# DavidPetrus/ood_object_detection

Measured on AMD Instinct MI355X. Metric: images/sec, tf_efficientdet_d0 640px bf16 inference + OOD score (DetBenchPredict end-to-end), higher is better.
Workload: dtype bf16; 1 GPU; tf_efficientdet_d0 640x640 batch=64/GPU C=90, DetBenchPredict: backbone+BiFPN+heads+OOD energy/max-logit+top-k(5000)+decode+hard NMS; global_batch=64, parallelism=image-sharded dp1, no collective, weights=seeded reference init, randomised BN stats, class bias 0, launch=hipgraph, images_in_flight=192

## Files before the change

ood_object_detection_amd/_lib.py:

```python
import ctypes
import os
import subprocess

_HERE = os.path.dirname(os.path.abspath(__file__))
LIB_PATH = os.path.join(_HERE, 'libeffdet_hip.so')
CSRC = os.path.join(_HERE, 'csrc')

_lib = None

LABEL_PAD = -2 ** 63

c_void_p, c_int, c_ll, c_float, c_double = ctypes.c_void_p, ctypes.c_int, ctypes.c_longlong, ctypes.c_float, ctypes.c_double
P = ctypes.POINTER

SIGNATURES = {
    'effdet_abi_version': (c_int, []),
    'effdet_last_error': (ctypes.c_char_p, []),
    'effdet_device_error': (c_int, [c_int]),
    'effdet_stem_conv': (c_int, [c_void_p, c_int, c_int, c_void_p, c_void_p, c_void_p, c_void_p, c_void_p,
                                 c_int, c_int, c_int, c_int]),
    'effdet_stem_dw_fused': (c_int, [c_void_p, c_int, c_int, c_void_p, c_void_p, c_void_p, c_void_p, c_void_p, c_void_p,
                                     c_void_p, c_void_p, c_void_p, c_int, c_int, c_int, c_int]),
    'effdet_resize_pad_u8': (c_int, [c_void_p, c_void_p, c_int, c_int, c_void_p, c_int, c_int, c_int, c_void_p, c_void_p, c_int,
                                     c_void_p, c_void_p, c_int, c_void_p, c_void_p]),
# ... 99 lines not shown
    'effdet_nms_soft_large': (c_int, [c_void_p, c_void_p, c_void_p, c_void_p, c_void_p, c_void_p, c_void_p, c_int, c_int,
                                      c_int, c_float, c_float, c_float, c_int, c_void_p, c_void_p, c_void_p, c_void_p, c_void_p]),
    'effdet_detection_loss_workspace_floats': (c_ll, [c_int, c_ll, c_int]),
    'effdet_detection_loss': (c_int, [c_void_p, c_int, c_void_p, c_void_p, c_void_p, c_void_p, c_void_p, c_int, c_ll, c_int,
                                      c_float, c_float, c_float, c_float, c_void_p, c_void_p, c_void_p, c_void_p, c_ll]),
    'effdet_label_anchors_workspace_bytes': (c_ll, [c_int, c_int, c_ll]),
    'effdet_label_anchors': (c_int, [c_void_p, c_void_p, c_void_p, c_void_p, c_int, c_int, c_ll, c_float, c_void_p, c_void_p,
                                     c_void_p, c_void_p, c_void_p, c_ll]),
    'effdet_label_anchors_rows': (c_int, [c_void_p, c_void_p, c_void_p, c_void_p, c_int, c_int, c_ll, c_float, c_void_p, c_void_p,
                                          c_void_p, c_void_p, c_void_p, c_ll]),
    'effdet_relabel_task_cls': (c_int, [c_void_p, c_void_p, c_void_p, c_int, c_int, c_ll, c_float]),
    'effdet_train_gemm_nt': (c_int, [c_void_p, c_void_p, c_ll, c_ll, c_ll, c_void_p, c_void_p, c_void_p, c_ll, c_ll, c_ll,
                                     c_ll, c_int, c_int, c_int, c_void_p]),
    'effdet_train_gemm_tn_workspace_floats': (c_ll, [c_ll, c_int, c_int]),
    'effdet_train_gemm_tn': (c_int, [c_void_p, c_void_p, c_ll, c_ll, c_ll, c_void_p, c_ll, c_ll, c_ll, c_ll, c_int, c_int,
                                     c_void_p, c_void_p, c_ll]),
    'effdet_train_reduce_mid': (c_int, [c_void_p, c_void_p, c_int, c_int, c_ll, c_void_p, c_int]),
    'effdet_train_dwconv_bwd_dx': (c_int, [c_void_p, c_void_p, c_void_p, c_void_p, c_int, c_int, c_int, c_int, c_int, c_int]),
    'effdet_train_dwconv_bwd_dw_workspace_floats': (c_ll, [c_int, c_int, c_int, c_int, c_int, c_int]),
    'effdet_train_dwconv_bwd_dw': (c_int, [c_void_p, c_void_p, c_void_p, c_void_p, c_int, c_int, c_int, c_int, c_int, c_int,
                                           c_void_p, c_ll, c_int]),
    'effdet_train_ew': (c_int, [c_void_p, c_int, c_void_p, c_void_p, c_void_p, c_void_p, c_void_p, c_void_p, c_void_p, c_void_p,
                                c_float, c_float, c_float, c_float, c_ll, c_int, c_ll, c_void_p, c_void_p]),
    'effdet_train_col_reduce_workspace_floats': (c_ll, [c_int, c_ll, c_int]),
    'effdet_train_col_reduce': (c_int, [c_void_p, c_int, c_void_p, c_void_p, c_void_p, c_int, c_ll, c_int, c_void_p, c_void_p, c_ll, c_float]),
    'effdet_train_spatial': (c_int, [c_void_p, c_int, c_void_p, c_void_p, c_void_p, c_int, c_int, c_int, c_int]),
    'effdet_train_im2col_stem': (c_int, [c_void_p, c_void_p, c_void_p, c_int, c_int, c_int]),
    'effdet_train_se_bwd': (c_int, [c_void_p, c_void_p, c_int, c_void_p, c_void_p, c_void_p, c_void_p, c_void_p, c_void_p, c_void_p,
                                    c_int, c_int, c_int]),
    'effdet_eval_match': (c_int, [c_void_p, c_void_p, c_void_p, c_void_p, c_void_p, c_int, c_int, c_int, c_int, c_float,
                                  c_void_p, c_void_p, c_void_p, c_void_p]),
    'effdet_eval_ap_workspace_bytes': (c_ll, [c_int]),
    'effdet_eval_ap': (c_int, [c_void_p, c_void_p, c_void_p, c_void_p, c_int, c_int, c_void_p, c_void_p, c_void_p, c_ll]),
    'effdet_eval_match_multi': (c_int, [c_void_p, c_void_p, c_void_p, c_void_p, c_void_p, c_void_p, c_int, c_int, c_int, c_int,
                                        c_void_p, c_int, c_void_p, c_void_p, c_void_p, c_void_p, c_void_p]),
    'effdet_eval_append': (c_int, [c_void_p, c_void_p, c_void_p, c_void_p, c_int, c_int, c_void_p, c_void_p, c_void_p, c_ll, c_void_p]),
    'effdet_eval_scale_sort_tile': (c_int, []),
    'effdet_eval_ap_sorted_workspace_bytes': (c_ll, [c_ll, c_int]),
    'effdet_eval_ap_sorted_offset': (c_ll, [c_ll, c_int, c_int]),
    'effdet_eval_ap_sorted_result_bytes': (c_ll, [c_int, c_int]),
    'effdet_eval_ap_sorted': (c_int, [c_void_p, c_void_p, c_void_p, c_void_p, c_ll, c_ll, c_void_p, c_int, c_int, c_void_p,
                                      c_void_p, c_void_p, c_void_p, c_ll, c_void_p]),
    'effdet_eval_open_words': (c_int, [c_void_p, c_void_p, c_void_p, c_void_p, c_void_p, c_int, c_int, c_int, c_int, c_void_p, c_int,
                                       c_void_p]),
    'effdet_eval_append_open': (c_int, [c_void_p, c_void_p, c_void_p, c_void_p, c_void_p, c_int, c_int, c_void_p, c_void_p, c_void_p,
                                        c_void_p, c_ll, c_void_p]),
    'effdet_eval_open_sorted_workspace_bytes': (c_ll, [c_ll, c_int]),
    'effdet_eval_open_sorted_offset': (c_ll, [c_ll, c_int, c_int]),
    'effdet_eval_open_sorted_result_bytes': (c_ll, [c_int, c_int]),
    'effdet_eval_open_sorted': (c_int, [c_void_p, c_void_p, c_void_p, c_void_p, c_void_p, c_ll, c_ll, c_void_p, c_int, c_int,
                                        c_void_p, c_void_p, c_void_p, c_double, c_void_p, c_ll, c_void_p]),
    'effdet_relabel_unknown': (c_int, [c_void_p, c_void_p, c_void_p, c_void_p, c_ll, c_ll, c_int, c_int, c_int, c_float, c_void_p,
                                       c_void_p]),
    'effdet_train_fold_bn': (c_int, [c_void_p, c_void_p, c_int, c_int, c_void_p, c_void_p, c_void_p, c_void_p, c_float,
                                     c_void_p, c_void_p, c_void_p, c_void_p, c_void_p, c_void_p]),
    'effdet_train_convbn_grads': (c_int, [c_void_p, c_void_p, c_int, c_int, c_int, c_void_p, c_void_p, c_void_p, c_void_p,
                                          c_void_p, c_void_p, c_void_p]),
    'effdet_train_bn_finalize': (c_int, [c_void_p, c_void_p, c_void_p, c_void_p, c_void_p, c_void_p, c_void_p, c_void_p, c_int, c_int,
                                         c_float, c_float, c_float, c_void_p, c_void_p, c_void_p]),
    'effdet_train_bn_bwd_prep': (c_int, [c_void_p, c_void_p, c_void_p, c_void_p, c_int, c_float, c_void_p, c_void_p, c_void_p, c_void_p]),
    'effdet_train_gemm_nt_levels': (c_int, [c_void_p, c_void_p, c_int, c_void_p, c_void_p, c_void_p, c_int, c_int, c_int, P(c_int), P(c_int),
                                            c_ll, c_ll, c_int, c_int, c_void_p]),
    'effdet_train_gemm_tn_levels': (c_int, [c_void_p, c_void_p, c_int, c_void_p, c_int, c_int, P(c_int), P(c_int), c_ll, c_ll, c_int, c_int,
                                            c_void_p, c_void_p, c_ll]),
    'effdet_train_levels_workspace_floats': (c_ll, [c_int, c_int, P(c_int), P(c_int), c_int]),
    'effdet_train_levels_dw': (c_int, [c_void_p, c_void_p, c_void_p, c_void_p, c_int, c_int, P(c_int), P(c_int), c_int, c_int]),
    'effdet_train_levels_dw_bwd_dw': (c_int, [c_void_p, c_void_p, c_void_p, c_void_p, c_int, c_int, P(c_int), P(c_int), c_int,
                                              c_void_p, c_ll, c_int]),
    'effdet_train_levels_col_reduce': (c_int, [c_void_p, c_int, c_void_p, c_void_p, c_void_p, c_void_p, P(c_float), c_int, c_int,
                                               P(c_int), P(c_int), c_int, c_void_p, c_void_p, c_ll]),
    'effdet_train_levels_bn_finalize': (c_int, [c_void_p, c_void_p, c_void_p, c_int, c_int, P(c_void_p), P(c_void_p), P(c_void_p),
                                                P(c_void_p), P(c_void_p), P(c_int), P(c_float), P(c_float), P(c_float), P(c_float),
                                                c_void_p, c_void_p, c_void_p, c_void_p]),
    'effdet_train_levels_bn_bwd_prep': (c_int, [c_void_p, c_void_p, c_void_p, P(c_float), c_int, c_int, c_void_p, c_void_p, c_void_p,
                                                c_void_p]),
    'effdet_train_levels_ew': (c_int, [c_void_p, c_int, c_void_p, c_void_p, c_void_p, c_void_p, c_void_p, c_void_p, c_void_p, c_void_p,
                                       c_void_p, P(c_int), c_int, c_int, P(c_int), P(c_int), c_int]),
    'effdet_train_fpn_weights': (c_int, [c_void_p, c_void_p, c_int, c_int, c_void_p]),
    'effdet_train_fpn_combine': (c_int, [c_void_p, c_int, P(c_void_p), P(c_int), P(c_int), c_int, c_void_p, c_void_p, c_void_p,
                                         c_int, c_int, c_int, c_int]),
    'effdet_train_fpn_dots_workspace_floats': (c_ll, [c_int, c_int, c_int, c_int]),
    'effdet_train_fpn_wgrad': (c_int, [c_void_p, c_int, P(c_void_p), P(c_int), P(c_int), c_int, c_void_p, c_void_p, c_void_p, c_void_p,
                                       c_void_p, c_void_p, c_int, c_int, c_int, c_int, c_void_p, c_ll]),
    'effdet_train_fpn_input_bwd': (c_int, [c_void_p, c_int, c_void_p, c_int, c_int, c_void_p, c_void_p, c_void_p, c_void_p, c_void_p,
                                           c_int, c_int, c_int, c_int]),
    'effdet_train_dwconv_fwd_parts': (c_int, [c_int, c_int, c_int, c_int, c_int]),
    'effdet_train_gemm_nt_plan_describe': (c_int, [c_ll, c_int, c_int, c_int, c_ll, c_ll, c_ll, c_int, c_ll, c_ll, c_ll, c_int, c_ll, c_int,
                                                   P(c_int), P(c_int), c_int]),
    'effdet_train_gemm_tn_plan_describe': (c_int, [c_ll, c_int, c_int, c_int, c_ll, c_ll, c_ll, c_int, c_ll, c_ll, c_ll, c_ll,
                                                   P(c_int), P(c_int), c_int]),
    'effdet_train_dwconv_plan_describe': (c_int, [c_int, c_int, c_int, c_int, c_int, c_int, c_int, P(c_int), c_int]),
    'effdet_train_dwconv_fwd': (c_int, [c_void_p, c_void_p, c_void_p, c_void_p, c_void_p, c_void_p, c_void_p, c_void_p,
                                        c_int, c_int, c_int, c_int, c_int, c_int]),
    'effdet_train_se_gate': (c_int, [c_void_p, c_void_p, c_int, c_int, c_void_p, c_void_p, c_void_p, c_void_p, c_void_p, c_void_p,
                                     c_int, c_int, c_int]),
    'effdet_train_gemm_nt_fused': (c_int, [c_void_p, c_void_p, c_void_p, c_ll, c_void_p, c_void_p, c_void_p, c_void_p, c_void_p,
                                           c_ll, c_int, c_int]),
    'effdet_train_gemm_tn_scaled': (c_int, [c_void_p, c_void_p, c_void_p, c_void_p, c_ll, c_ll, c_int, c_int, c_void_p, c_void_p, c_ll]),
    'effdet_train_dwconv_bwd_dx_silu': (c_int, [c_void_p, c_void_p, c_void_p, c_void_p, c_void_p, c_int, c_int, c_int, c_int, c_int, c_int]),
    'effdet_train_gemm_nt_relu': (c_int, [c_void_p, c_void_p, c_void_p, c_void_p, c_ll, c_int, c_int]),
    'effdet_train_gemm_nt_mask': (c_int, [c_void_p, c_void_p, c_void_p, c_void_p, c_void_p, c_ll, c_int, c_int]),
    'effdet_train_relu_mask': (c_int, [c_void_p, c_void_p, c_void_p, c_void_p, c_ll]),
    'effdet_train_prep_table': (c_int, [c_void_p, c_void_p, c_int, c_ll]),
    'effdet_train_grads_table': (c_int, [c_void_p, c_void_p, c_int, c_int]),
    'effdet_train_bn_var_finalize': (c_int, [c_void_p, c_void_p, c_void_p, c_ll, c_int, c_void_p, c_void_p, c_void_p, c_void_p, c_void_p,
                                             c_float, c_float, c_float, c_void_p, c_void_p, c_void_p, c_void_p, c_ll]),
    'effdet_train_bn_bwd_sums': (c_int, [c_void_p, c_void_p, c_void_p, c_void_p, c_void_p, c_ll, c_int, c_void_p, c_void_p, c_ll]),
    'effdet_gather_ood': (c_int, [c_void_p, c_void_p, c_void_p, c_void_p, c_void_p, c_ll, c_int, c_int, c_int,
                                  c_void_p, c_void_p, c_void_p]),
    'effdet_episode_select': (c_int, [c_void_p, c_int, c_int, P(c_void_p), P(c_ll), P(c_int), P(c_int), P(c_void_p)]),
    'effdet_episode_feed': (c_int, [c_void_p, c_int, c_int, P(c_void_p), P(c_ll), P(c_void_p), P(c_ll), P(c_void_p), P(c_int), P(c_int),
                                    c_void_p, c_void_p, c_int, c_void_p, c_int, c_int, c_int, c_int, c_int, c_void_p, c_void_p]),
    'effdet_episode_cluster_workspace_floats': (c_ll, [c_int, c_int, c_int]),
    'effdet_episode_cluster': (c_int, [c_void_p, c_void_p, c_void_p, c_int, c_int, c_int, c_float, c_float, c_void_p, c_int, c_float,
                                       c_int, c_void_p, c_ll, c_void_p, c_void_p, c_void_p, c_void_p, c_void_p, c_void_p, c_void_p,
                                       c_void_p, c_void_p, c_void_p, c_void_p]),
    'effdet_episode_proj_loss_workspace_floats': (c_ll, [c_int, c_int, c_int]),
    'effdet_episode_proj_loss': (c_int, [c_void_p, c_void_p, c_void_p, c_void_p, c_int, c_int, c_int, c_ll, c_void_p, c_float, c_float,
                                         c_void_p, c_void_p, c_void_p, c_void_p, c_void_p, c_int, c_int, c_float, c_void_p, c_ll,
                                         c_void_p, c_void_p, c_void_p, c_void_p]),
    'effdet_episode_proj_loss_backward': (c_int, [c_void_p, c_void_p, c_void_p, c_void_p, c_int, c_int, c_int, c_ll, c_void_p, c_float,
                                                  c_float, c_void_p, c_void_p, c_void_p, c_void_p, c_void_p, c_int, c_int, c_float,
                                                  c_void_p, c_void_p, c_ll, c_void_p, c_void_p, c_void_p]),
    'effdet_episode_supp_loss_workspace_floats': (c_ll, [c_int, c_int, c_int]),
    'effdet_episode_supp_loss': (c_int, [c_void_p, c_void_p, c_void_p, c_void_p, c_int, c_int, c_int, c_float, c_float, c_void_p,
                                         c_void_p, c_void_p, c_void_p, c_void_p, c_int, c_void_p, c_ll, c_void_p, c_void_p]),
    'effdet_episode_supp_loss_backward': (c_int, [c_void_p, c_void_p, c_void_p, c_void_p, c_int, c_int, c_int, c_float, c_float,
                                                  c_void_p, c_void_p, c_void_p, c_void_p, c_void_p, c_int, c_int, c_void_p, c_void_p,
                                                  c_ll, c_void_p, c_void_p, c_void_p, c_void_p]),
    'effdet_episode_supp_loss_backward2': (c_int, [c_void_p, c_void_p, c_void_p, c_void_p, c_int, c_int, c_int, c_float, c_float,
                                                   c_void_p, c_void_p, c_void_p, c_void_p, c_void_p, c_int, c_int, c_void_p, c_void_p,
                                                   c_void_p, c_void_p, c_void_p, c_void_p, c_void_p, c_ll, c_void_p, c_void_p,
                                                   c_void_p, c_void_p, c_void_p]),
    'effdet_inner_update_max_tensors': (c_int, []),
    'effdet_inner_update_max_step_sizes': (c_int, []),
    'effdet_inner_update_workspace_doubles': (c_ll, [c_int, P(c_ll)]),
    'effdet_inner_update': (c_int, [c_void_p, c_int, P(c_void_p), P(c_void_p), P(c_void_p), P(c_ll), P(c_int), c_int, P(c_void_p),
                                    P(c_float)]),
    'effdet_inner_update_backward': (c_int, [c_void_p, c_int, P(c_void_p), P(c_void_p), P(c_void_p), P(c_ll), P(c_int), c_int,
                                             P(c_void_p), P(c_float), c_void_p, c_ll, c_int, c_void_p]),
}


def build(verbose=False):
    jobs = str(min(8, os.cpu_count() or 1))
    r = subprocess.run(['make', '-C', CSRC, '-j', jobs], capture_output=not verbose, text=True)
    if r.returncode != 0:
        raise RuntimeError('building libeffdet_hip.so failed:\n%s\n%s' % (r.stdout, r.stderr))
    return LIB_PATH


TEST_VARIANTS = {
    'spin0': ('mbconv_wide', '-DWIDE_SPIN_LIMIT=0'),
}


def build_test_variants(verbose=False):
    paths = []
    for tag, (unit, defs) in TEST_VARIANTS.items():
        r = subprocess.run(['make', '-C', CSRC, 'variant', 'TAG=' + tag, 'UNIT=' + unit, 'VDEFS=' + defs], capture_output=not verbose, text=True)
        if r.returncode != 0:
            raise RuntimeError('building the %s variant failed:\n%s\n%s' % (tag, r.stdout, r.stderr))
        paths.append(os.path.join(_HERE, 'libeffdet_hip_%s.so' % tag))
    return paths


def load():
    global _lib
    if _lib is not None:
        return _lib
    import torch
    if not os.path.exists(LIB_PATH):
        raise RuntimeError('%s is missing - run `python -c "import __graft_entry__ as g; g.build()"` '
                           '(there is no CPU fallback for the HIP path)' % LIB_PATH)
    lib = ctypes.CDLL(LIB_PATH)
    for name, (res, args) in SIGNATURES.items():
        fn = getattr(lib, name)
        fn.restype = res
        fn.argtypes = args
    if lib.effdet_abi_version() != 1:
        raise RuntimeError('libeffdet_hip.so ABI version mismatch')
    _lib = lib
    return lib


def check(rc, what):
    if rc != 0:
        detail = ''
        if rc == -5 and _lib is not None:
            detail = ' (%s)' % (_lib.effdet_last_error() or b'').decode()
        raise RuntimeError('%s failed with code %d%s' % (what, rc, detail))
```

ood_object_detection_amd/csrc/sepconv.hip:

```cpp
#include "common.h"
#include <type_traits>

namespace {

struct SepInput {
    const void* ptr; long long image_stride;
    int H, W; int mode;
    int pad_t, pad_l;
};
struct SepLevel {
    int H, W, tiles_x, tiles_y, tile_begin, affine_row;
    SepInput in[3];
    void* out; long long out_image_stride;
    long long ood_off;
    int in_affine_row;
    void* dw_out; long long dw_out_image_stride;
};
struct SepArgs {
    int nlevels; SepLevel lv[5];
    int n_in, fuse_mode;
    float fw[3]; float fden;
    float fwn[3];
    int vec_ok;
    int out_f32;
    int pre_act, post_act;
    const float* dw_w;
    const void* pw_w;
    const float* scale; const float* shift;
    int F, N;
    int ood_classes, num_anchors;
    float* ood_energy; float* ood_maxlogit; long long ood_image_stride;
    const float* in_scale; const float* in_shift;
    float* stat_partial;
    int tiles_total;
};

constexpr int FC = 64;



template <typename T> struct Raw8 { u32x4 v[sizeof(T) == 2 ? 1 : 2]; };
template <typename T> DEV Raw8<T> load_raw8(const T* p) {
    Raw8<T> r;
    r.v[0] = *reinterpret_cast<const u32x4*>(p);
    if constexpr (sizeof(T) == 4) r.v[1] = *(reinterpret_cast<const u32x4*>(p) + 1);
    return r;
}
template <typename T> DEV F8 unpack8(const Raw8<T>& r) {
    F8 o;
    if constexpr (IsPair<T>::value) {
        return pair_join8(r.v[0], r.v[1]);
    } else if constexpr (sizeof(T) == 2) {
        const bf16x8 a = __builtin_bit_cast(bf16x8, r.v[0]);
#pragma unroll
        for (int e = 0; e < 8; ++e) o.v[e] = (float)a[e];
    } else {
        const f32x4 a = __builtin_bit_cast(f32x4, r.v[0]), b = __builtin_bit_cast(f32x4, r.v[1]);
#pragma unroll
        for (int e = 0; e < 4; ++e) { o.v[e] = a[e]; o.v[4 + e] = b[e]; }
    }
    return o;
}
template <typename T> DEV Raw8<T> pack8(const F8& f) {
    Raw8<T> r;
    if constexpr (IsPair<T>::value) {
        pair_split8(f, r.v[0], r.v[1]);
    } else if constexpr (sizeof(T) == 2) {
        bf16x8 a;
#pragma unroll
        for (int e = 0; e < 8; ++e) a[e] = (bf16_t)f.v[e];
        r.v[0] = __builtin_bit_cast(u32x4, a);
    } else {
        r.v[0] = __builtin_bit_cast(u32x4, f32x4{f.v[0], f.v[1], f.v[2], f.v[3]});
        r.v[1] = __builtin_bit_cast(u32x4, f32x4{f.v[4], f.v[5], f.v[6], f.v[7]});
    }
    return r;
}

template <typename T>
DEV Raw8<T> fetch_input(const T* base, const SepInput& in, int y, int x, int F, int c) {
    if (in.mode != 2) {
        const int sh = in.mode == 1 ? 1 : 0;
        return load_raw8<T>(base + ((y >> sh) * in.W + (x >> sh)) * F + c);
    }
    F8 m = f8_fill(-INFINITY);
#pragma unroll
    for (int ky = 0; ky < 3; ++ky) {
        const int iy = 2 * y + ky - in.pad_t;
        const int iyc = iy < 0 ? 0 : (iy >= in.H ? in.H - 1 : iy);
#pragma unroll
        for (int kx = 0; kx < 3; ++kx) {
            const int ix = 2 * x + kx - in.pad_l;
            const int ixc = ix < 0 ? 0 : (ix >= in.W ? in.W - 1 : ix);
            const F8 v = load8<T>(base + (iyc * in.W + ixc) * F + c);
            const bool inside = iy == iyc && ix == ixc;
#pragma unroll
            for (int e = 0; e < 8; ++e) m.v[e] = fmaxf(m.v[e], inside ? v.v[e] : -INFINITY);
        }
    }
    return pack8<T>(m);
}

template <typename T>
DEV void store_piece(T* dst, const float (&v)[8], int nvalid, bool vec_ok) {
    if constexpr (IsPair<T>::value) {
        typedef unsigned u32x4_a4 __attribute__((ext_vector_type(4), aligned(4)));
        F8 f;
#pragma unroll
        for (int e = 0; e < 8; ++e) f.v[e] = v[e];
        u32x4 hi, lo;
        pair_split8(f, hi, lo);
        if (nvalid >= 8) {
            *reinterpret_cast<u32x4_a4*>(dst) = hi;
            *(reinterpret_cast<u32x4_a4*>(dst) + 1) = lo;
        }
    } else
    if (vec_ok && nvalid >= 8) {
        if constexpr (sizeof(T) == 2) {
            typedef unsigned u32x4_a4 __attribute__((ext_vector_type(4), aligned(4)));
            bf16x8 a;
#pragma unroll
            for (int e = 0; e < 8; ++e) a[e] = (bf16_t)v[e];
            *reinterpret_cast<u32x4_a4*>(dst) = __builtin_bit_cast(u32x4, a);
        } else {
            typedef float f32x4_a4 __attribute__((ext_vector_type(4), aligned(4)));
            *reinterpret_cast<f32x4_a4*>(dst) = f32x4{v[0], v[1], v[2], v[3]};
            *reinterpret_cast<f32x4_a4*>(dst + 4) = f32x4{v[4], v[5], v[6], v[7]};
        }
    } else {
        if constexpr (!IsPair<T>::value) {
#pragma unroll
            for (int e = 0; e < 8; ++e)
                if (e < nvalid) dst[e] = from_f<T>(v[e]);
        }
    }
}

template <typename T, int TH, int TW, int BN, bool OOD, int NTH, int FT, bool META = false, int NIN = 3, bool BST = false>
__global__ __launch_bounds__(NTH, NTH == 512 ? (FT == 64 && !OOD && !META && !IsPair<T>::value ? 8 : 4) : 2) void sepconv_kernel(SepArgs p) {
    constexpr int BM = TH * TW;
    constexpr int HW_ = (TH + 2) * (TW + 2);
    constexpr int NWAVE = NTH / 64;
    constexpr int WPT = BM / (16 * NWAVE);
    constexpr int NT = BN / 16;
    constexpr int NP = NT / 2;
    static_assert(NT % 2 == 0 && WPT >= 1, "tile shape");
    extern __shared__ __attribute__((aligned(16))) char lds[];

    const int F = FT ? FT : p.F, N = p.N;
    const int fbytes = F * (int)sizeof(T);
    constexpr int PB = OpGeom<T>::PIECE, CHB = OpGeom<T>::CHUNK;
    const int nkc = (fbytes + CHB - 1) / CHB;
    const int arow = nkc * CHB + 16;
    constexpr bool MF = IsFast<T>::value && TW == 16 && NTH == 512;
    constexpr int HROW = FC + (MF ? 16 / (int)sizeof(T) : 0);
    constexpr int HALO_BYTES = HW_ * HROW * (int)sizeof(T);
    constexpr bool CP = MF && FT == 64 && !META;
    const int r0 = CP ? (HALO_BYTES > (BM + BN) * arow ? HALO_BYTES : (BM + BN) * arow)
                      : (HALO_BYTES > BN * arow ? HALO_BYTES : BN * arow);
    char* halo = lds;
    char* Wt = CP ? lds + BM * arow : lds;
    char* At = CP ? lds : lds + r0;
    float* dww = reinterpret_cast<float*>(CP ? lds + r0 : At + BM * arow);
    float* cs = dww + 9 * F;

    const int tid = threadIdx.x, lane = tid & 63, wave = tid >> 6;
    const int b = blockIdx.y;
    int li = 0;
#pragma unroll
    for (int q = 1; q < 5; ++q) if (q < p.nlevels && (int)blockIdx.x >= p.lv[q].tile_begin) li = q;
    const SepLevel& L = p.lv[li];
    const int t = blockIdx.x - L.tile_begin;
    const int y0 = (t / L.tiles_x) * TH, x0 = (t % L.tiles_x) * TW;
    const int H = L.H, W = L.W;

    constexpr int DPC = (9 * 128 + NTH - 1) / NTH;
    const bool d_pref = 9 * F <= DPC * NTH;
    float dpre[DPC];
#pragma unroll
    for (int q = 0; q < DPC; ++q) {
        const int i = tid + NTH * q;
        dpre[q] = (d_pref && i < 9 * F) ? p.dw_w[i] : 0.f;
    }
    if (nkc * CHB > fbytes) {
        const int padb = nkc * CHB - fbytes;
        for (int i = tid; i < BM * (padb / 16); i += NTH) {
            const int row = i / (padb / 16), piece = i % (padb / 16);
            *reinterpret_cast<u32x4*>(At + row * arow + fbytes + piece * 16) = u32x4{0u, 0u, 0u, 0u};
// ... 449 lines not shown
                                stq[i][J][e] = q;
                            }
                        }
                    }
                    if constexpr (OOD) {
                        if (!group_full) {
#pragma unroll
                            for (int e = 0; e < 8; ++e) if (e >= nvalid) vals[J][e] = -INFINITY;
                        }
                        m = fmaxf(m, fmaxf(fmaxf(fmaxf(vals[J][0], vals[J][1]), fmaxf(vals[J][2], vals[J][3])),
                                           fmaxf(fmaxf(vals[J][4], vals[J][5]), fmaxf(vals[J][6], vals[J][7]))));
                    }
                }
            }
            if constexpr (OOD) {
                m = fmaxf(m, __shfl_xor(m, 16, 64));
                m = fmaxf(m, __shfl_xor(m, 32, 64));
                const float tm = (m == -INFINITY) ? 0.f : m;
#pragma unroll
                for (int J = 0; J < NP; ++J) {
                    if (J < njp) {
                        if constexpr (IsFast<T>::value) {
                            const float tl = tm * LOG2E;
#pragma unroll
                            for (int e = 0; e < 8; ++e) ssum += __builtin_amdgcn_exp2f(fmaf(vals[J][e], LOG2E, -tl));
                        } else {
#pragma unroll
                            for (int e = 0; e < 8; ++e) ssum += (vals[J][e] == -INFINITY) ? 0.f : expf(vals[J][e] - tm);
                        }
                    }
                }
                ssum += __shfl_xor(ssum, 16, 64);
                ssum += __shfl_xor(ssum, 32, 64);
                const int sc = ch % subs;
                float pm = sc == 0 ? -INFINITY : run_m[i], ps = sc == 0 ? 0.f : run_s[i];
                if (m != -INFINITY) {
                    const float nm = fmaxf(pm, m);
                    ps = (pm == -INFINITY ? 0.f : ps * exp_t<T>(pm - nm)) + ssum * exp_t<T>(m - nm);
                    pm = nm;
                }
                run_m[i] = pm; run_s[i] = ps;
                if constexpr (BST) {
                    constexpr int OOB = 0x7FFFFFF0;
                    const int a = ch / subs;
                    const int eo = (sc == subs - 1 && pix_in[i] && fpiece == 0) ? ((pix_off[i] / N) * p.num_anchors + a) * 4 : OOB;
                    __builtin_amdgcn_raw_buffer_store_b32(__builtin_bit_cast(unsigned, -(pm + logf(ps))), ers, eo, 0, 0);
                    __builtin_amdgcn_raw_buffer_store_b32(__builtin_bit_cast(unsigned, pm), mrs, eo, 0, 0);
                } else
                if (sc == subs - 1 && pix_in[i] && fpiece == 0) {
                    const int a = ch / subs;
                    const long long idx = (long long)b * p.ood_image_stride + L.ood_off +
                                          (long long)(pix_off[i] / N) * p.num_anchors + a;
                    p.ood_energy[idx] = -(pm + logf(ps));
                    p.ood_maxlogit[idx] = pm;
                }
            }
        }
        if constexpr (META) {
            if (p.stat_partial != nullptr) {
                float* piv = cs;
                float* sst = cs + 2 * BN;
                if (wave == 0 && frow == 0) {
#pragma unroll
                    for (int J = 0; J < NP; ++J)
#pragma unroll
                        for (int e = 0; e < 8; ++e) piv[32 * J + 8 * fpiece + e] = stq[0][J][e];
                }
                __syncthreads();
#pragma unroll
                for (int J = 0; J < NP; ++J)
#pragma unroll
                    for (int e = 0; e < 8; ++e) {
                        const float pv = piv[32 * J + 8 * fpiece + e];
                        float a = 0.f, q = 0.f;
#pragma unroll
                        for (int i = 0; i < WPT; ++i) {
                            const float d = pix_in[i] ? stq[i][J][e] - pv : 0.f;
                            a += d; q += d * d;
                        }
#pragma unroll
                        for (int o = 1; o < 16; o <<= 1) { a += __shfl_xor(a, o, 64); q += __shfl_xor(q, o, 64); }
                        if (frow == 0) { sst[(wave * 2 + 0) * BN + 32 * J + 8 * fpiece + e] = a; sst[(wave * 2 + 1) * BN + 32 * J + 8 * fpiece + e] = q; }
                    }
                __syncthreads();
                if (tid < 2 * BN) {
                    const int which = tid / BN, n = tid % BN;
                    float tot = 0.f;
                    for (int w = 0; w < NWAVE; ++w) tot += sst[(w * 2 + which) * BN + n];
                    if (n < n_count) {
                        float* row = p.stat_partial + (((long long)b * p.tiles_total + blockIdx.x) * 3) * N + n_begin + n;
                        row[(1 + which) * (long long)N] = tot;
                        if (which == 0) row[0] = piv[n];
                    }
                }
            }
        }
    }
}

template <typename T, int TH, int TW, int BN>
size_t sep_lds_bytes(int F, bool cp = false) {
    constexpr int BM = TH * TW;
    constexpr int HW_ = (TH + 2) * (TW + 2);
    const int nkc = (F * (int)sizeof(T) + OpGeom<T>::CHUNK - 1) / OpGeom<T>::CHUNK;
    const int arow = nkc * OpGeom<T>::CHUNK + 16;
    const size_t halo = (size_t)HW_ * (FC + (IsFast<T>::value && TW == 16 ? 16 / (int)sizeof(T) : 0)) * sizeof(T);
    const size_t wt = (size_t)BN * arow;
    if (cp) return (halo > wt + (size_t)BM * arow ? halo : wt + (size_t)BM * arow) + (size_t)9 * F * 4 + (size_t)2 * BN * 4;
    return (halo > wt ? halo : wt) + (size_t)BM * arow + (size_t)9 * F * 4 + (size_t)2 * BN * 4;
}

template <typename T, int TH, int TW, int BN, bool OOD, int NTH, int FT, bool META = false, int NIN = 3, bool BST = false>
int launch_sep(hipStream_t st, SepArgs& a, int B) {
    int tiles = 0;
    for (int i = 0; i < a.nlevels; ++i) {
        a.lv[i].tiles_x = (a.lv[i].W + TW - 1) / TW;
        a.lv[i].tiles_y = (a.lv[i].H + TH - 1) / TH;
        a.lv[i].tile_begin = tiles;
        tiles += a.lv[i].tiles_x * a.lv[i].tiles_y;
    }
    const size_t lds = sep_lds_bytes<T, TH, TW, BN>(a.F, IsFast<T>::value && TW == 16 && NTH == 512 && FT == 64 && !META) + (META ? (size_t)(NTH / 64) * 2 * BN * 4 : 0);
    if (lds > 160 * 1024) return EFFDET_EINVAL;
    a.tiles_total = tiles;
    auto kern = sepconv_kernel<T, TH, TW, BN, OOD, NTH, FT, META, NIN, BST>;
    if (lds > 64 * 1024) {
        static bool attr_done = false;
        if (!attr_done) {
            if (hipFuncSetAttribute(reinterpret_cast<const void*>(kern), hipFuncAttributeMaxDynamicSharedMemorySize, 160 * 1024) != hipSuccess)
                return EFFDET_ELAUNCH;
            attr_done = true;
        }
    }
    hipLaunchKernelGGL(kern, dim3(tiles, B), dim3(NTH), lds, st, a);
    return effdet_check_launch();
}

constexpr int BST_TH = 8;
template <typename T, int TH, int TW, int NTH, int FT>
int dispatch_sep_f(hipStream_t st, SepArgs& a, int B) {
    if (a.ood_classes > 0) {
        if constexpr (FT == 0) {
            if (sep_lds_bytes<T, TH, TW, 96>(a.F) > 160 * 1024) return launch_sep<T, TH, TW, 64, true, NTH, FT>(st, a, B);
        }
        if constexpr (IsPair<T>::value && NTH == 512) {
            if (a.out_f32 && a.ood_classes % 2 == 0 && a.ood_classes <= 96 && a.F <= 64 && a.scale == nullptr && !a.post_act)
                return launch_sep<T, BST_TH, TW, 96, true, NTH, FT, false, 3, true>(st, a, B);
        }
        if constexpr (sizeof(T) == 2 && NTH == 512) {
            if (a.vec_ok && !a.out_f32 && a.ood_classes % 2 == 0 && a.ood_classes <= 96 && a.F <= 64 && a.scale == nullptr && !a.post_act)
                return launch_sep<T, BST_TH, TW, 96, true, NTH, FT, false, 3, true>(st, a, B);
        }
        return launch_sep<T, TH, TW, 96, true, NTH, FT>(st, a, B);
    }
    if (FT == 64 && a.n_in == 1) return launch_sep<T, TH, TW, 64, false, NTH, FT, false, 1>(st, a, B);
    return launch_sep<T, TH, TW, 64, false, NTH, FT>(st, a, B);
}

template <typename T, int TH, int TW, int NTH>
int dispatch_sep(hipStream_t st, SepArgs& a, int B) {
    switch (a.F) {
        case 64:  return dispatch_sep_f<T, TH, TW, NTH, 64>(st, a, B);
        case 88:  return dispatch_sep_f<T, TH, TW, NTH, 88>(st, a, B);
        case 112: return dispatch_sep_f<T, TH, TW, NTH, 112>(st, a, B);
        case 160: return dispatch_sep_f<T, TH, TW, NTH, 160>(st, a, B);
        case 224: return dispatch_sep_f<T, TH, TW, NTH, 224>(st, a, B);
        default:  return dispatch_sep_f<T, TH, TW, NTH, 0>(st, a, B);
    }
}

template <int FT>
int dispatch_sep_pair_8x8(hipStream_t st, SepArgs& a, int B) {
    if (a.ood_classes > 0) {
        if constexpr (FT == 0) {
            if (sep_lds_bytes<bf16p_t, 8, 8, 96>(a.F) > 160 * 1024) return launch_sep<bf16p_t, 8, 8, 64, true, 256, 0>(st, a, B);
        }
        return launch_sep<bf16p_t, 8, 8, 96, true, 256, FT>(st, a, B);
    }
    return launch_sep<bf16p_t, 8, 8, 64, false, 256, FT>(st, a, B);
}

}

namespace {
struct MetaExtra {
    const float* in_scale; const float* in_shift; const int* in_affine_row;
    float* stat_partial;
    void* const* dw_out; const long long* dw_out_image_stride;
};
}

static int sepconv_common(
    const MetaExtra* meta,
    void* stream, int dtype, int B, int nlevels,
    const int* level_hw,
    int n_in,
    const void* const* in_ptr,
    const long long* in_image_stride,
    const int* in_hw,
    const int* in_mode,
    int fuse_mode, const float* fuse_w, float fuse_den, int pre_act,
    const float* dw_w, const void* pw_w, const float* scale, const float* shift,
    const int* affine_row,
    int post_act, int F, int N,
    void* const* out_ptr, const long long* out_image_stride,
    int ood_classes, int num_anchors, float* ood_energy, float* ood_maxlogit,
    long long ood_image_stride, const long long* ood_level_off) {
    if (nlevels < 1 || nlevels > 5 || n_in < 1 || n_in > 3 || B <= 0) return EFFDET_EINVAL;
    if (!level_hw || !in_ptr || !in_image_stride || !in_hw || !in_mode || !dw_w || !pw_w || !shift || !affine_row ||
        !out_ptr || !out_image_stride) return EFFDET_EINVAL;
    const int sym = take_pad_flag(dtype);
    if (dtype != 0 && dtype != 1 && dtype != 2 && dtype != 3 && dtype != 6) return EFFDET_EINVAL;
    const int out_f32 = (dtype == 3 || dtype == 6) ? 1 : 0;
    dtype = dtype == 3 ? 1 : (dtype == 6 ? 2 : dtype);
    if (dtype == 2 && (meta || (!out_f32 && N % 8))) return EFFDET_EINVAL;
    if (F <= 0 || F % 8 || N <= 0 || fuse_mode < 0 || fuse_mode > 2) return EFFDET_EINVAL;
    if (fuse_mode != 0 && !fuse_w) return EFFDET_EINVAL;
    if (fuse_mode == 0 && n_in != 1) return EFFDET_EINVAL;
    if (ood_classes > 0) {
        if (!ood_energy || !ood_maxlogit || !ood_level_off || num_anchors <= 0 || num_anchors * ood_classes != N) return EFFDET_EINVAL;
    }
    SepArgs a;
    a.nlevels = nlevels; a.n_in = n_in; a.fuse_mode = fuse_mode; a.fden = fuse_den;
    for (int i = 0; i < 3; ++i) a.fw[i] = (fuse_mode != 0 && i < n_in) ? fuse_w[i] : 0.f;
    for (int i = 0; i < 3; ++i) a.fwn[i] = fuse_mode == 1 ? a.fw[i] / fuse_den : a.fw[i];
    const size_t esz = (dtype == 0 || out_f32) ? 4 : 2;
    a.out_f32 = out_f32;
    a.vec_ok = ((size_t)N * esz) % 4 == 0 && (ood_classes <= 0 || ((size_t)ood_classes * esz) % 4 == 0);
    a.pre_act = pre_act; a.post_act = post_act; a.dw_w = dw_w; a.pw_w = pw_w; a.scale = scale; a.shift = shift;
    a.F = F; a.N = N; a.ood_classes = ood_classes > 0 ? ood_classes : 0; a.num_anchors = num_anchors;
    a.ood_energy = ood_energy; a.ood_maxlogit = ood_maxlogit; a.ood_image_stride = ood_image_stride;
    a.in_scale = meta ? meta->in_scale : nullptr; a.in_shift = meta ? meta->in_shift : nullptr;
    a.stat_partial = meta ? meta->stat_partial : nullptr; a.tiles_total = 0;
    if (meta && ((meta->in_scale != nullptr) != (meta->in_shift != nullptr) || (meta->in_scale && !meta->in_affine_row))) return EFFDET_EINVAL;
    for (int l = 0; l < nlevels; ++l) {
        SepLevel& L = a.lv[l];
        L.in_affine_row = (meta && meta->in_affine_row) ? meta->in_affine_row[l] : 0;
        L.dw_out = (meta && meta->dw_out) ? meta->dw_out[l] : nullptr;
        L.dw_out_image_stride = (meta && meta->dw_out_image_stride) ? meta->dw_out_image_stride[l] : 0;
        if (L.dw_out && reinterpret_cast<uintptr_t>(L.dw_out) % 16) return EFFDET_EINVAL;
        L.H = level_hw[2 * l]; L.W = level_hw[2 * l + 1];
        if (L.H <= 0 || L.W <= 0) return EFFDET_EINVAL;
        L.affine_row = affine_row[l];
        L.out = out_ptr[l]; L.out_image_stride = out_image_stride[l];
        L.ood_off = (ood_classes > 0) ? ood_level_off[l] : 0;
        if (!L.out) return EFFDET_EINVAL;
        if (reinterpret_cast<uintptr_t>(L.out) % 16 || ((size_t)L.out_image_stride * esz) % 4) a.vec_ok = 0;
        for (int i = 0; i < n_in; ++i) {
            SepInput& I = L.in[i];
            I.ptr = in_ptr[l * n_in + i]; I.image_stride = in_image_stride[l * n_in + i];
            I.H = in_hw[(l * n_in + i) * 2]; I.W = in_hw[(l * n_in + i) * 2 + 1];
            I.mode = in_mode[l * n_in + i];
            I.pad_t = I.pad_l = 0;
            if (!I.ptr) return EFFDET_EINVAL;
            if (I.mode == 0) { if (I.H != L.H || I.W != L.W) return EFFDET_EINVAL; }
            else if (I.mode == 1) { if (I.H * 2 != L.H || I.W * 2 != L.W) return EFFDET_EINVAL; }
            else if (I.mode == 2) {
                if (same_out(I.H, 2) != L.H || same_out(I.W, 2) != L.W) return EFFDET_EINVAL;
                I.pad_t = pad_before(I.H, 3, 2, sym); I.pad_l = pad_before(I.W, 3, 2, sym);
            } else return EFFDET_EINVAL;
        }
    }
    hipStream_t st = reinterpret_cast<hipStream_t>(stream);
    if (meta) {
        if (ood_classes > 0 || fuse_mode != 0 || out_f32 || scale != nullptr) return EFFDET_EINVAL;
        return dtype == 0 ? launch_sep<float, 8, 8, 64, false, 256, 0, true>(st, a, B)
                          : launch_sep<bf16_t, 8, 16, 64, false, 512, 0, true>(st, a, B);
    }
    if (dtype == 0) return dispatch_sep<float, 8, 8, 256>(st, a, B);
    if (dtype == 2) {
        for (int l = 0; l < nlevels; ++l) {
            if (!out_f32 && (reinterpret_cast<uintptr_t>(a.lv[l].out) % 16 || a.lv[l].out_image_stride % 4)) return EFFDET_EINVAL;
            for (int i = 0; i < n_in; ++i)
                if (reinterpret_cast<uintptr_t>(a.lv[l].in[i].ptr) % 16 || a.lv[l].in[i].image_stride % 4) return EFFDET_EINVAL;
        }
        if (sep_lds_bytes<bf16p_t, 8, 16, 64>(F) <= 160 * 1024) return dispatch_sep<bf16p_t, 8, 16, 512>(st, a, B);
        return F == 224 ? dispatch_sep_pair_8x8<224>(st, a, B) : dispatch_sep_pair_8x8<0>(st, a, B);
    }
    return dispatch_sep<bf16_t, 8, 16, 512>(st, a, B);
}

extern "C" int effdet_sepconv_fused(
    void* stream, int dtype, int B, int nlevels, const int* level_hw, int n_in,
    const void* const* in_ptr, const long long* in_image_stride, const int* in_hw, const int* in_mode,
    int fuse_mode, const float* fuse_w, float fuse_den, int pre_act,
    const float* dw_w, const void* pw_w, const float* scale, const float* shift, const int* affine_row,
    int post_act, int F, int N, void* const* out_ptr, const long long* out_image_stride,
    int ood_classes, int num_anchors, float* ood_energy, float* ood_maxlogit,
    long long ood_image_stride, const long long* ood_level_off) {
    EFFDET_ENTER();
    return sepconv_common(nullptr, stream, dtype, B, nlevels, level_hw, n_in, in_ptr, in_image_stride, in_hw, in_mode,
                          fuse_mode, fuse_w, fuse_den, pre_act, dw_w, pw_w, scale, shift, affine_row, post_act, F, N,
                          out_ptr, out_image_stride, ood_classes, num_anchors, ood_energy, ood_maxlogit, ood_image_stride, ood_level_off);
}

extern "C" int effdet_sepconv_meta(
    void* stream, int dtype, int B, int nlevels, const int* level_hw,
    const void* const* in_ptr, const long long* in_image_stride,
    const float* in_scale, const float* in_shift, const int* in_affine_row, int pre_act,
    const float* dw_w, const void* pw_w, const float* bias, int F, int N,
    void* const* out_ptr, const long long* out_image_stride,
    float* stat_partial, void* const* dw_out, const long long* dw_out_image_stride) {
    EFFDET_ENTER();
    if (nlevels < 1 || nlevels > 5 || !level_hw) return EFFDET_EINVAL;
    int in_hw[10], in_mode[5], arow[5];
    for (int l = 0; l < nlevels; ++l) { in_hw[2 * l] = level_hw[2 * l]; in_hw[2 * l + 1] = level_hw[2 * l + 1]; in_mode[l] = 0; arow[l] = 0; }
    MetaExtra m{in_scale, in_shift, in_affine_row, stat_partial, dw_out, dw_out_image_stride};
// ... 74 lines not shown
```

Baseline: 16930 images/sec.

## Add rolling-row-buffer separable conv kernel for 64-channel bf16 layers

Adds a new separable-conv kernel for bf16 inputs with F=64 and single-input, non-OOD cases. Each wave sweeps a 16-pixel strip down a band of rows and keeps a three-row ring buffer in LDS, so each input row is loaded once and reused across the vertical taps. The next rows are prefetched into registers while the current row is computed. Both the depthwise 3x3 (built as diagonal MFMA fragments) and the pointwise 1x1 run on the matrix units, with a fused affine and SiLU epilogue. Band height is picked per level from a cost model of halo overhead; the tradeoff is fewer blocks than the tiled kernel and extra register and LDS pressure.

```diff
diff --git a/ood_object_detection_amd/_lib.py b/ood_object_detection_amd/_lib.py
--- a/ood_object_detection_amd/_lib.py
+++ b/ood_object_detection_amd/_lib.py
@@ -275,7 +275,16 @@
 
 TEST_VARIANTS = {
     'spin0': ('mbconv_wide', '-DWIDE_SPIN_LIMIT=0'),
+    'septile': ('sepconv', '-DSEP_ROLL_OFF'),
 }
+
+SEPCONV_ROLL_STRIP = 16
+SEPCONV_ROLL_BAND_MAX = 16
+
+
+def sepconv_roll_plan(W):
+    cost = lambda R: -(-W // R) * (R + 5)
+    return SEPCONV_ROLL_STRIP, min(range(1, SEPCONV_ROLL_BAND_MAX + 1), key=lambda R: (cost(R), R))
 
 
 def build_test_variants(verbose=False):
diff --git a/ood_object_detection_amd/csrc/sepconv.h b/ood_object_detection_amd/csrc/sepconv.h
--- /dev/null
+++ b/ood_object_detection_amd/csrc/sepconv.h
@@ -0,0 +1,38 @@
+#pragma once
+#include "common.h"
+
+struct SepInput {
+    const void* ptr; long long image_stride;
+    int H, W; int mode;
+    int pad_t, pad_l;
+};
+struct SepLevel {
+    int H, W, tiles_x, tiles_y, tile_begin, affine_row;
+    SepInput in[3];
+    void* out; long long out_image_stride;
+    long long ood_off;
+    int in_affine_row;
+    void* dw_out; long long dw_out_image_stride;
+};
+struct SepArgs {
+    int nlevels; SepLevel lv[5];
+    int n_in, fuse_mode;
+    float fw[3]; float fden;
+    float fwn[3];
+    int vec_ok;
+    int out_f32;
+    int pre_act, post_act;
+    const float* dw_w;
+    const void* pw_w;
+    const float* scale; const float* shift;
+    int F, N;
+    int ood_classes, num_anchors;
+    float* ood_energy; float* ood_maxlogit; long long ood_image_stride;
+    const float* in_scale; const float* in_shift;
+    float* stat_partial;
+    int tiles_total;
+};
+
+__attribute__((visibility("hidden"))) void effdet_sepconv_roll_plan(int W, int* strip_px, int* band_rows);
+__attribute__((visibility("hidden"))) bool effdet_sepconv_roll_applies(const SepArgs& a);
+__attribute__((visibility("hidden"))) int effdet_sepconv_roll_launch(hipStream_t st, const SepArgs& a, int B);
diff --git a/ood_object_detection_amd/csrc/sepconv.hip b/ood_object_detection_amd/csrc/sepconv.hip
--- a/ood_object_detection_amd/csrc/sepconv.hip
+++ b/ood_object_detection_amd/csrc/sepconv.hip
@@ -1,39 +1,7 @@
-#include "common.h"
+#include "sepconv.h"
 #include <type_traits>
 
 namespace {
-
-struct SepInput {
-    const void* ptr; long long image_stride;
-    int H, W; int mode;
-    int pad_t, pad_l;
-};
-struct SepLevel {
-    int H, W, tiles_x, tiles_y, tile_begin, affine_row;
-    SepInput in[3];
-    void* out; long long out_image_stride;
-    long long ood_off;
-    int in_affine_row;
-    void* dw_out; long long dw_out_image_stride;
-};
-struct SepArgs {
-    int nlevels; SepLevel lv[5];
-    int n_in, fuse_mode;
-    float fw[3]; float fden;
-    float fwn[3];
-    int vec_ok;
-    int out_f32;
-    int pre_act, post_act;
-    const float* dw_w;
-    const void* pw_w;
-    const float* scale; const float* shift;
-    int F, N;
-    int ood_classes, num_anchors;
-    float* ood_energy; float* ood_maxlogit; long long ood_image_stride;
-    const float* in_scale; const float* in_shift;
-    float* stat_partial;
-    int tiles_total;
-};
 
 constexpr int FC = 64;
 
@@ -789,6 +757,11 @@
         }
         return launch_sep<T, TH, TW, 96, true, NTH, FT>(st, a, B);
     }
+#ifndef SEP_ROLL_OFF
+    if constexpr (std::is_same<T, bf16_t>::value && FT == 64) {
+        if (effdet_sepconv_roll_applies(a)) return effdet_sepconv_roll_launch(st, a, B);
+    }
+#endif
     if (FT == 64 && a.n_in == 1) return launch_sep<T, TH, TW, 64, false, NTH, FT, false, 1>(st, a, B);
     return launch_sep<T, TH, TW, 64, false, NTH, FT>(st, a, B);
 }
diff --git a/ood_object_detection_amd/csrc/sepconv_roll.hip b/ood_object_detection_amd/csrc/sepconv_roll.hip
--- /dev/null
+++ b/ood_object_detection_amd/csrc/sepconv_roll.hip
@@ -0,0 +1,312 @@
+#include "sepconv.h"
+
+#ifndef SEPR_STRIP_TILES
+#define SEPR_STRIP_TILES 1
+#endif
+#ifndef SEPR_WAVES
+#define SEPR_WAVES 3
+#endif
+#ifndef SEPR_WAVES_TAIL
+#define SEPR_WAVES_TAIL 2
+#endif
+#ifndef SEPR_BAND_MAX
+#define SEPR_BAND_MAX 16
+#endif
+
+namespace {
+
+struct RollGeo { int item_begin[6]; int nstrips[5]; int band[5]; };
+
+constexpr int WPG = 4;
+constexpr int PXB = 144;
+
+constexpr int roll_wave_lds(int ns) { return 3 * (16 * ns + 2) * PXB + ns * 16 * PXB; }
+
+template <int NS, bool ACT, bool OF32, bool TAIL>
+__global__ __launch_bounds__(64 * WPG, NS == 1 ? (TAIL ? SEPR_WAVES_TAIL : SEPR_WAVES) : 2) void sepconv_roll_kernel(SepArgs p, RollGeo g) {
+    extern __shared__ __attribute__((aligned(16))) char lds[];
+    typedef bf16_t T;
+    constexpr int RPX = 16 * NS + 2;
+    constexpr int ROWB = RPX * PXB;
+    constexpr int NL = (RPX * 8 + 63) / 64;
+    constexpr int OOB = 0x7FFFFFF0;
+    constexpr int OOBS = 0x40000000;
+    constexpr int ESZ = OF32 ? 4 : 2;
+    const int lane = threadIdx.x & 63, wave = __builtin_amdgcn_readfirstlane(threadIdx.x >> 6);
+    const int item = blockIdx.x * WPG + wave;
+    if (item >= g.item_begin[p.nlevels]) return;
+    int li = 0;
+#pragma unroll
+    for (int q = 1; q < 5; ++q) if (q < p.nlevels && item >= g.item_begin[q]) li = q;
+    const SepLevel& L = p.lv[li];
+    const int H = L.H, W = L.W, N = p.N;
+    const int b = blockIdx.y;
+    const int qi = item - g.item_begin[li];
+    const int strip = qi % g.nstrips[li], band = qi / g.nstrips[li];
+    const int x0 = strip * 16 * NS;
+    const int yb = band * g.band[li], ye = min(H, yb + g.band[li]);
+    const int frow = lane & 15, fp = lane >> 4;
+    char* const ring = lds + wave * roll_wave_lds(NS);
+    char* const ast = ring + 3 * ROWB;
+    auto aff = [&](int k) { return reinterpret_cast<float*>(ring + k * PXB + 128); };
+
+    Frag<T> wf[4][2];
+#pragma unroll
+    for (int j = 0; j < 4; ++j) {
+        const int co = 32 * (j >> 1) + 8 * (frow >> 2) + 4 * (j & 1) + (frow & 3);
+        const unsigned keep = co < N ? 0xFFFFFFFFu : 0u;
+#pragma unroll
+        for (int kc = 0; kc < 2; ++kc) {
+            const u32x4 v = *reinterpret_cast<const u32x4*>(reinterpret_cast<const char*>(p.pw_w) + (co < N ? co : 0) * 128 + kc * 64 + fp * 16);
+            wf[j][kc].v = __builtin_bit_cast(bf16x8, v & u32x4{keep, keep, keep, keep});
+        }
+    }
+    static_assert(3 * RPX >= 32, "pad bytes for the affine constants");
+    {
+        const int cc = lane < N ? lane : 0;
+        const float* srow = p.scale ? p.scale : p.shift;
+        const float tv = p.shift[(long long)L.affine_row * N + cc], sv = srow[(long long)L.affine_row * N + cc];
+        aff(lane >> 2)[lane & 3] = p.scale ? sv : 1.0f;
+        aff(16 + (lane >> 2))[lane & 3] = tv;
+    }
+    const int hi = fp >> 1;
+    const bool dactive = (fp & 1) == (frow >> 3);
+    const int dq = (frow & 7) >> 1;
+    unsigned abits[4][5];
+#pragma unroll
+    for (int j = 0; j < 4; ++j)
+#pragma unroll
+        for (int pr = 0; pr < 5; ++pr) {
+            const int t = 2 * pr + hi;
+            const float wv = p.dw_w[(t < 9 ? t : 0) * 64 + 16 * j + frow];
+            const unsigned on = (dactive && t < 9) ? 0xFFFFFFFFu : 0u;
+            abits[j][pr] = ((unsigned)__builtin_bit_cast(unsigned short, (bf16_t)wv) << (16 * (frow & 1))) & on;
+        }
+    auto diag = [&](int j, int pr) {
+        unsigned bits = abits[j][pr];
+        asm volatile("" : "+v"(bits));
+        const u32x4 fr = {dq == 0 ? bits : 0u, dq == 1 ? bits : 0u, dq == 2 ? bits : 0u, dq == 3 ? bits : 0u};
+        Frag<T> af;
+        af.v = __builtin_bit_cast(bf16x8, fr);
+        return af;
+    };
+
+    int voff[NL];
+    char* wdst[NL];
+#pragma unroll
+    for (int q = 0; q < NL; ++q) {
+        const int i = lane + 64 * q < RPX * 8 ? lane + 64 * q : RPX * 8 - 1, x = x0 - 1 + (i >> 3);
+        voff[q] = (x >= 0 && x < W) ? x * 128 + (i & 7) * 16 : OOB;
+        wdst[q] = ring + (i >> 3) * PXB + (i & 7) * 16;
+    }
+    const SepInput& I = L.in[0];
+    const __amdgpu_buffer_rsrc_t irs = __builtin_amdgcn_make_buffer_rsrc(
+        const_cast<char*>(reinterpret_cast<const char*>(I.ptr)) + (long long)b * I.image_stride * 2, 0, H * W * 128, 0x00020000);
+    const __amdgpu_buffer_rsrc_t ors = __builtin_amdgcn_make_buffer_rsrc(
+        reinterpret_cast<char*>(L.out) + (long long)b * L.out_image_stride * ESZ, 0, H * W * N * ESZ, 0x00020000);
+    auto load_row = [&](int iy, u32x4 (&dst)[NL]) {
+        const bool rowin = iy >= 0 && iy < H;
+        const int soff = (rowin ? iy : 0) * W * 128;
+#pragma unroll
+        for (int q = 0; q < NL; ++q) dst[q] = __builtin_amdgcn_raw_buffer_load_b128(irs, rowin ? voff[q] : OOB, soff, 0);
+    };
+    auto put_row = [&](int slot, const u32x4 (&src)[NL]) {
+#pragma unroll
+        for (int q = 0; q < NL; ++q) *reinterpret_cast<u32x4*>(wdst[q] + slot * ROWB) = src[q];
+    };
+    const char* const dl0 = ring + frow * PXB + (fp & 1) * 16;
+    const char* const dsame = dl0 + hi * PXB;
+    const char* const dnw = dl0 + hi * (ROWB - 2 * PXB);
+    const char* const dwr = dl0 + (1 - hi) * (2 * ROWB + 2 * PXB);
+    int ooff[NS][2];
+#pragma unroll
+    for (int t = 0; t < NS; ++t)
+#pragma unroll
+        for (int J = 0; J < 2; ++J) {
+            const int x = x0 + 16 * t + frow, c = 32 * J + 8 * fp;
+            ooff[t][J] = (x < W && N - c >= 8) ? (x * N + c) * ESZ : OOBS;
+        }
+    const int tJ = N >> 5, tn4 = N & 4, tn1 = N & 3;
+    int toff[TAIL ? NS : 1];
+    if constexpr (TAIL) {
+#pragma unroll
+        for (int t = 0; t < NS; ++t) {
+            const int x = x0 + 16 * t + frow;
+            toff[t] = (x < W && fp == ((N & 31) >> 3)) ? (x * N + (N & ~7)) * ESZ : OOBS;
+        }
+    }
+
+    u32x4 xq[2][NL];
+    {
+        u32x4 xa[NL], xb[NL];
+        load_row(yb - 1, xa); load_row(yb, xb); load_row(yb + 1, xq[0]); load_row(yb + 2, xq[1]);
+        put_row(0, xa); put_row(1, xb);
+    }
+    int y = yb;
+    auto step = [&](auto PHC, auto QC) {
+        constexpr int PH = decltype(PHC)::value, Q = decltype(QC)::value;
+        put_row((PH + 2) % 3, xq[Q]);
+        load_row(y + 3, xq[Q]);
+        const int orow = y * W * N * ESZ;
+#pragma unroll
+        for (int t = 0; t < NS; ++t) {
+#pragma unroll
+            for (int j = 0; j < 4; ++j) {
+                f32x4 acc = {0.f, 0.f, 0.f, 0.f};
+#pragma unroll
+                for (int pr = 0; pr < 5; ++pr) {
+                    const int t0 = 2 * pr, t1 = 2 * pr + 1 < 9 ? 2 * pr + 1 : 0;
+                    const int offa = ((PH + t0 / 3) % 3) * ROWB + (t0 % 3) * PXB;
+                    const int offb = ((PH + t1 / 3) % 3) * ROWB + (t1 % 3) * PXB;
+                    const char* src = offb - offa == PXB ? dsame + offa
+                                    : offb - offa == ROWB - 2 * PXB ? dnw + offa
+                                    : dwr + offb;
+                    mma_chunk(diag(j, pr), ld_frag<T>(src + t * 16 * PXB + 32 * j), acc);
+                }
+                row_store4<T>(ast + (16 * t + frow) * PXB, 16 * j + 4 * fp, acc);
+            }
+            Frag<T> xb[2];
+#pragma unroll
+            for (int kc = 0; kc < 2; ++kc) xb[kc] = ld_frag<T>(ast + (16 * t + frow) * PXB + kc * 64 + fp * 16);
+            f32x4 acc[4];
+#pragma unroll
+            for (int j = 0; j < 4; ++j) acc[j] = f32x4{0.f, 0.f, 0.f, 0.f};
+#pragma unroll
+            for (int kc = 0; kc < 2; ++kc)
+#pragma unroll
+                for (int j = 0; j < 4; ++j) mma_chunk(wf[j][kc], xb[kc], acc[j]);
+            float tv[8];
+#pragma unroll
+            for (int J = 0; J < 2; ++J) {
+                const f32x4 s0 = *reinterpret_cast<const f32x4*>(aff(8 * J + 2 * fp)), s1 = *reinterpret_cast<const f32x4*>(aff(8 * J + 2 * fp + 1));
+                const f32x4 h0 = *reinterpret_cast<const f32x4*>(aff(16 + 8 * J + 2 * fp)), h1 = *reinterpret_cast<const f32x4*>(aff(16 + 8 * J + 2 * fp + 1));
+                float vals[8];
+#pragma unroll
+                for (int r = 0; r < 4; ++r) {
+                    float a0 = fmaf(acc[2 * J][r], s0[r], h0[r]);
+                    float a1 = fmaf(acc[2 * J + 1][r], s1[r], h1[r]);
+                    if constexpr (ACT) { a0 = silu_t<T>(a0); a1 = silu_t<T>(a1); }
+                    vals[r] = a0; vals[4 + r] = a1;
+                }
+                if constexpr (OF32) {
+                    __builtin_amdgcn_raw_buffer_store_b128(__builtin_bit_cast(u32x4, f32x4{vals[0], vals[1], vals[2], vals[3]}), ors, ooff[t][J] + orow, 0, 0);
+                    __builtin_amdgcn_raw_buffer_store_b128(__builtin_bit_cast(u32x4, f32x4{vals[4], vals[5], vals[6], vals[7]}), ors, ooff[t][J] + 16 + orow, 0, 0);
+                } else {
+                    bf16x8 a8;
+#pragma unroll
+                    for (int e = 0; e < 8; ++e) a8[e] = (bf16_t)vals[e];
+                    __builtin_amdgcn_raw_buffer_store_b128(__builtin_bit_cast(u32x4, a8), ors, ooff[t][J] + orow, 0, 0);
+                }
+                if constexpr (TAIL) {
+#pragma unroll
+                    for (int e = 0; e < 8; ++e) tv[e] = (J == 0 || tJ == J) ? vals[e] : tv[e];
+                }
+            }
+            if constexpr (TAIL) {
+                const int o4 = tn4 ? toff[t] : OOBS;
+                if constexpr (OF32) {
+                    __builtin_amdgcn_raw_buffer_store_b128(__builtin_bit_cast(u32x4, f32x4{tv[0], tv[1], tv[2], tv[3]}), ors, o4 + orow, 0, 0);
+                } else {
+                    const bf16x4 a4 = {(bf16_t)tv[0], (bf16_t)tv[1], (bf16_t)tv[2], (bf16_t)tv[3]};
+                    __builtin_amdgcn_raw_buffer_store_b64(__builtin_bit_cast(u32x2, a4), ors, o4 + orow, 0, 0);
+                }
+#pragma unroll
+                for (int e = 0; e < 3; ++e) {
+                    const float v = tn4 ? tv[4 + e] : tv[e];
+                    const int off = (e < tn1 && toff[t] != OOBS) ? toff[t] + ((tn4 ? 4 : 0) + e) * ESZ : OOBS;
+                    if constexpr (OF32) __builtin_amdgcn_raw_buffer_store_b32(__builtin_bit_cast(unsigned, v), ors, off + orow, 0, 0);
+                    else __builtin_amdgcn_raw_buffer_store_b16(__builtin_bit_cast(unsigned short, (bf16_t)v), ors, off + orow, 0, 0);
+                }
+            }
+        }
+        ++y;
+    };
+    for (;;) {
+        step(IntC<0>{}, IntC<0>{}); if (y >= ye) break;
+        step(IntC<1>{}, IntC<1>{}); if (y >= ye) break;
+        step(IntC<2>{}, IntC<0>{}); if (y >= ye) break;
+        step(IntC<0>{}, IntC<1>{}); if (y >= ye) break;
+        step(IntC<1>{}, IntC<0>{}); if (y >= ye) break;
+        step(IntC<2>{}, IntC<1>{}); if (y >= ye) break;
+    }
+}
+
+constexpr bool sep_roll_pairs_ok(int rowb) {
+    for (int ph = 0; ph < 3; ++ph)
+        for (int pr = 0; pr < 5; ++pr) {
+            const int t0 = 2 * pr, t1 = 2 * pr + 1 < 9 ? 2 * pr + 1 : 0;
+            const int offa = ((ph + t0 / 3) % 3) * rowb + (t0 % 3) * PXB, offb = ((ph + t1 / 3) % 3) * rowb + (t1 % 3) * PXB;
+            if (offb - offa != PXB && offb - offa != rowb - 2 * PXB && offa - offb != 2 * rowb + 2 * PXB) return false;
+        }
+    return true;
+}
+static_assert(sep_roll_pairs_ok((16 * SEPR_STRIP_TILES + 2) * PXB), "tap pair addressing");
+
+template <int NS, bool ACT, bool OF32, bool TAIL>
+int launch_roll(hipStream_t st, const SepArgs& a, const RollGeo& g, int B) {
+    constexpr int lds = WPG * roll_wave_lds(NS);
+    static_assert(lds <= 160 * 1024, "LDS");
+    auto kern = sepconv_roll_kernel<NS, ACT, OF32, TAIL>;
+    if (lds > 64 * 1024) {
+        static bool attr_done = false;
+        if (!attr_done) {
+            if (hipFuncSetAttribute(reinterpret_cast<const void*>(kern), hipFuncAttributeMaxDynamicSharedMemorySize, lds) != hipSuccess)
+                return EFFDET_ELAUNCH;
+            attr_done = true;
+        }
+    }
+    const int items = g.item_begin[a.nlevels];
+    hipLaunchKernelGGL(kern, dim3((items + WPG - 1) / WPG, B), dim3(64 * WPG), lds, st, a, g);
+    return effdet_check_launch();
+}
+
+}
+
+void effdet_sepconv_roll_plan(int W, int* strip_px, int* band_rows) {
+    int best = 1, best_cost = 0x7FFFFFFF;
+    for (int R = 1; R <= SEPR_BAND_MAX; ++R) {
+        const int cost = ((W + R - 1) / R) * (R + 5);
+        if (cost < best_cost) { best = R; best_cost = cost; }
+    }
+    *strip_px = 16 * SEPR_STRIP_TILES;
+    *band_rows = best;
+}
+
+bool effdet_sepconv_roll_applies(const SepArgs& a) {
+    if (a.F != 64 || a.N < 1 || a.N > 64 || a.n_in != 1 || a.fuse_mode != 0 || a.pre_act || a.ood_classes > 0 || !a.vec_ok) return false;
+    if (a.in_scale || a.stat_partial) return false;
+    for (int l = 0; l < a.nlevels; ++l) {
+        if ((long long)a.lv[l].H * a.lv[l].W > (1 << 21)) return false;
+        if (a.lv[l].in[0].mode != 0 || a.lv[l].dw_out) return false;
+    }
+    return true;
+}
+
+int effdet_sepconv_roll_launch(hipStream_t st, const SepArgs& a, int B) {
+    RollGeo g;
+    int items = 0;
+    for (int l = 0; l < 5; ++l) {
+        g.item_begin[l] = items;
+        g.nstrips[l] = g.band[l] = 1;
+        if (l >= a.nlevels) continue;
+        int strip, R;
+        effdet_sepconv_roll_plan(a.lv[l].W, &strip, &R);
+        g.nstrips[l] = (a.lv[l].W + strip - 1) / strip;
+        g.band[l] = R;
+        items += g.nstrips[l] * ((a.lv[l].H + R - 1) / R);
+    }
+    g.item_begin[5] = items;
+    for (int l = a.nlevels; l < 5; ++l) g.item_begin[l] = items;
+    constexpr int NS = SEPR_STRIP_TILES;
+    const int sel = (a.post_act ? 4 : 0) | (a.out_f32 ? 2 : 0) | (a.N % 8 ? 1 : 0);
+    switch (sel) {
+        case 0: return launch_roll<NS, false, false, false>(st, a, g, B);
+        case 1: return launch_roll<NS, false, false, true>(st, a, g, B);
+        case 2: return launch_roll<NS, false, true, false>(st, a, g, B);
+        case 3: return launch_roll<NS, false, true, true>(st, a, g, B);
+        case 4: return launch_roll<NS, true, false, false>(st, a, g, B);
+        case 5: return launch_roll<NS, true, false, true>(st, a, g, B);
+        case 6: return launch_roll<NS, true, true, false>(st, a, g, B);
+        default: return launch_roll<NS, true, true, true>(st, a, g, B);
+    }
+}
```

Measured after the change: 16810 images/sec (median of 2 runs). No clear change (-0.7%).
